# thu-nics/Rad-NeRF

Measured on AMD Instinct MI355X. Metric: million samples/s fwd+bwd, 8192 rays, model_zoo_size=2; rgb L∞ vs ref, higher is better.
Workload: dtype f16/f32

## Files before the change

rad-nerf_amd/csrc/field.hip:

```cpp
#include "rn_field.h"
#include "rn_bin.h"
#include "rn_merge.h"
#include "rn_gradform.h"
#pragma clang fp contract(off)

static int g_field_dbg = 0;
__device__ unsigned long long g_rn_cyc[8];

namespace {

template <int MODE, int CACHE>
__global__ void __launch_bounds__(256, FWD_MIN_WAVES)
k_field_fwd(FieldArgs a) {
    __shared__ __attribute__((aligned(16))) rn_half sW[FIELD_FWD_FRAGS * RN_FRAG_HALFS];
    __shared__ LvTab sT;
    const int k = blockIdx.y;
    rn_block_copy16(sW, a.frags + (size_t)k * FIELD_FRAGS * RN_FRAG_HALFS,
                    FIELD_FWD_FRAGS * RN_FRAG_BYTES);
    lv_stage(sT, a.gm);
    __syncthreads();
    int64_t base, n;
    sample_range(a, MODE, k, base, n);
    const int64_t n_tiles = (n + 31) / 32;
    const int waves = blockDim.x / RN_WAVE;
// ... 789 lines not shown
    auto eighth_g = [&](int e) -> float* {
        return e < 4 ? reinterpret_cast<float*>(sImg) + e * EB
                     : reinterpret_cast<float*>(sW) + (e - 4) * EB;
    };
    static_assert(4 * W2_RING_WORDS * 4 <= BWD_WAVES * SC_STREAMS * 3 * SC_RING * 4, "rings");
    static_assert(4 * EB * 4 + 4 * W2_RING_WORDS * 4 <= BWD_WAVES * 2 * RN_IMG_HALFS * 2,
                  "eighths 0-3 + rings in the image region");
    static_assert(4 * EB * 4 <= FIELD_FRAGS * RN_FRAG_HALFS * 2, "eighths 4-7 in the weights");
    uint32_t* ring2 = wid < 4 ? sRing + wid * W2_RING_WORDS
                              : reinterpret_cast<uint32_t*>(sImg) + 4 * EB +
                                    (wid - 4) * W2_RING_WORDS;
    float* const wG = eighth_g(rn_lane() >> 3);
    float* const wU = wG + MB_WIN * SG_STRIDE;
    bool sw_ok = false;

    f32x16 accA = rn_zero16(), accB = rn_zero16();
    DwScale cur = {0.f, 0.f};
    int cur_k = -1;
    uint64_t cyc[8] = {0, 0, 0, 0, 0, 0, 0, 0};
    float* park = m.park + (size_t)blockIdx.x * K * BWD_WAVES * 2048 + wid * 2048;
    float* rows = m.scratch + (size_t)blockIdx.x * m.rows_cap * MB_ROW;
    const __amdgpu_buffer_rsrc_t rows_rs = rn_rsrc(rows, (uint32_t)m.rows_cap * MB_ROW * 4u);
    int n_local = 0;
    int ticket = 0, n_chunks = 0;
    if (threadIdx.x == 0) {
        n_chunks = m.queue[1];
        ticket = DET ? (int)blockIdx.x : atomicAdd(m.queue, 1);
    }
    if (threadIdx.x < K) sCh[2 + 3 * MB_KMAX + threadIdx.x] = a.seg_base[threadIdx.x];

    for (;;) {
        __syncthreads();
        if (threadIdx.x == 0) {
            const int ch = ticket;
            ticket = DET ? (ch < n_chunks ? ch + (int)gridDim.x : ch) : atomicAdd(m.queue, 1);
            int4 d[CH_DESC / 4];
            if (ch < n_chunks) {
#pragma unroll
                for (int q = 0; q < CH_DESC / 4; ++q)
                    d[q] = reinterpret_cast<const int4*>(m.desc + (size_t)ch * CH_DESC)[q];
            }
            const int32_t* di = reinterpret_cast<const int32_t*>(d);
            sCh[0] = ch < n_chunks ? di[CH_R0] : B; sCh[1] = ch < n_chunks ? di[CH_R1] : B;
            int roff = 0;
            for (int k = 0; k < K; ++k) {
                const int nk = ch < n_chunks ? di[ch_count(k)] : 0;
                sCh[2 + k] = di[ch_first(k)]; sCh[2 + MB_KMAX + k] = nk;
                sCh[2 + 2 * MB_KMAX + k] = roff;
                roff += nk;
            }
        }
        __syncthreads();
        const int r0 = sCh[0], r1 = sCh[1];
        if (r0 >= B) break;
        const bool rev = n_local & 1;
        ++n_local;
        constexpr int RAYS_LDS = BWD_WAVES * SC_STREAMS * 3 * SC_RING / 6;
        const int nr_lds = r1 - r0 <= RAYS_LDS ? r1 - r0 : 0;
        float* sRays = reinterpret_cast<float*>(sRing);
        for (int i = threadIdx.x; i < 6 * nr_lds; i += blockDim.x) {
            const int q = i / 6, cc = i - 6 * q;
            sRays[i] = cc < 3 ? a.rays_o[3 * (r0 + q) + cc] : a.rays_d[3 * (r0 + q) + cc - 3];
        }
        __syncthreads();

        const bool prof = ABL && (rn_dbg(dbg) & 4096);
        uint64_t tp0 = prof ? __builtin_amdgcn_s_memtime() : 0;
        for (int kk = 0; kk < K; ++kk) {
            const int k = rev ? K - 1 - kk : kk;
            const int a_k = sCh[2 + k], n_k = sCh[2 + MB_KMAX + k], roff = sCh[2 + 2 * MB_KMAX + k];
            if (n_k == 0) continue;
            uint64_t ts0 = prof ? __builtin_amdgcn_s_memtime() : 0;
            if (k != cur_k || !sw_ok) {
                constexpr int WV = (FIELD_FRAGS * RN_FRAG_BYTES / 16 + BWD_WAVES * RN_WAVE - 1) /
                                   (BWD_WAVES * RN_WAVE);
// ... 384 lines not shown
                      gb_pool_pages >= 1),
          "binned mode needs scale, stats, the encoding cache and the page pool");
    for (int l = 0; binned && l < RN_L; ++l)
        CHECK(level_hsize[l] <= (1u << GB_IDX_BITS) &&
              level_hsize[l] <= ((uint32_t)GB_MAX_BINS << GB_SLICE_BITS),
              "binned mode: a level has more than 2^20 entries");
    CHECK(fx_mode != GM_FX_REDO || (fx_redo && fx_scale && feat_cache),
          "fixed-point redo needs the redo flag, the step's scales and the encoding cache");
    CHECK(!(igrad_lo && fx_mode), "integer and fixed-point modes are exclusive");
    CHECK(n_rays >= 1 && n_models >= 1 && n_models <= MB_KMAX && blocks >= 1 &&
          max_samples >= 1 && max_chunk >= 1, "bad sizes");
    CHECK(scratch_rows >= (int64_t)max_chunk + (int64_t)n_models * max_samples,
          "scratch_rows must be >= max_chunk + n_models * max_samples");
    CHECK(ts && ray_of && rays_o && rays_d && seg_base && seg_count && mstart && perm &&
          chunk_desc && queue && grid_f16 && level_offset && level_hsize && level_res &&
          level_scale && xyz_min && extent && frags && dL_dsigma && dL_drgb && grid_grad && dw &&
          scratch && park, "null pointer");
    CHECK(fx_mode != GM_FX ||
          2ull * ((uint64_t)level_offset[RN_L - 1] + level_hsize[RN_L - 1]) <= (1ull << 28),
          "fixed-point mode: the grid has more than 2^28 gradient elements");
#undef CHECK
    FieldArgs a{};
    field_args_grid(a, grid_f16, level_offset, level_hsize, level_res, level_scale, xyz_min, extent,
                    frags);
    field_args_compact(a, ts, ray_of, rays_o, rays_d, seg_base, seg_count);
    a.dsigma = dL_dsigma; a.drgb = dL_drgb; a.grid_grad = grid_grad; a.dw = dw;
    a.feat = (rn_half*)feat_cache;
    MergeArgs m{};
    m.mstart = mstart; m.perm = perm; m.desc = chunk_desc; m.queue = queue; m.scratch = scratch;
    m.park = park; m.rows_cap = (int)scratch_rows; m.n_rays = (int)n_rays; m.n_models = n_models;
    hipStream_t st = (hipStream_t)stream;
    const size_t slots = (size_t)blocks * n_models * FIELD_PARAMS * sizeof(float);
    if (det) RN_CHECK_HIP_AS(who, hipMemsetAsync(dw, 0, slots, st), "dw_part reset");
    else RN_CHECK_HIP_AS(who, hipMemsetAsync(queue, 0, sizeof(int32_t), st), "ticket reset");
    IntGrad G{};
    if (igrad_lo) {
        G.bytes = 2 * a.grid_bytes;
        G.lo_ptr = igrad_lo; G.carry_ptr = igrad_carry; G.scale_ptr = igrad_scale;
    }
    if (binned) {
        RN_CHECK_HIP_AS(who, hipMemsetAsync(gb_ctl, 0, GB_CTL_RESET_BYTES, st), "page pool reset");
        G.ctl = (GbCtl*)gb_ctl; G.page_meta = gb_page_meta; G.pages = gb_pages;
        G.pool_pages = (uint32_t)gb_pool_pages;
    }
    FxGrad F{};
    F.acc = fx_acc; F.scale = fx_scale; F.redo = fx_redo;
    if (FxStats* S = reinterpret_cast<FxStats*>(fx_stats)) {
        F.vmax = S->vmax; F.qsum = S->qsum; F.wq = S->wq;
    }
    const int gm = fx_mode ? fx_mode : (igrad_lo ? GM_INT : GM_F32);
    const bool abl = RN_ABL && a.dbg && !det && gm != GM_INT && gm != GM_FX_REDO;
    if (abl) launch_bwd_merged<RN_ABL != 0, 0>(gm, blocks, st, a, m, G, F);
    else if (!det) launch_bwd_merged<false, 0>(gm, blocks, st, a, m, G, F);
    else launch_bwd_merged<false, 1>(gm, blocks, st, a, m, G, F);
    RN_CHECK_LAUNCH_AS(who);
    return 0;
}

extern "C" {
int rn_field_bwd_merged(const float* ts, const int32_t* ray_of, const float* rays_o,
                        const float* rays_d, const int32_t* seg_base, const int32_t* seg_count,
                        const int32_t* mstart, const int32_t* perm, const int32_t* chunk_desc,
                        int32_t* queue, int64_t n_rays, int32_t n_models, int32_t max_samples,
                        const void* grid_f16, const uint32_t* level_offset,
                        const uint32_t* level_hsize, const uint32_t* level_res,
                        const float* level_scale, const float* xyz_min, const float* extent,
                        const void* frags, const float* dL_dsigma, const float* dL_drgb,
// ... 43 lines not shown
```

rad-nerf_amd/csrc/field_grad.hip:

```cpp
#include "rn_field.h"
#include "rn_bin.h"
#include "rn_gradform.h"
#pragma clang fp contract(off)

namespace {

__global__ void __launch_bounds__(256)
k_seed_max(const int32_t* __restrict__ seg_base, const int32_t* __restrict__ seg_count,
           const float* __restrict__ sigma, const float* __restrict__ dsigma,
           const float* __restrict__ drgb, uint32_t* __restrict__ mbits) {
    const int k = blockIdx.y;
    const int64_t base = seg_base[k], n = seg_count[k];
    float mx = 0.f;
    for (int64_t i = (int64_t)blockIdx.x * blockDim.x + threadIdx.x; i < n;
         i += (int64_t)gridDim.x * blockDim.x) {
        const int64_t s = base + i;
        mx = fmaxf(mx, fabsf(dsigma[s] * sigma[s]));
        mx = fmaxf(mx, fmaxf(fabsf(drgb[3 * s]), fmaxf(fabsf(drgb[3 * s + 1]), fabsf(drgb[3 * s + 2]))));
    }
    mx = rn_wave_max(mx);
    if (rn_lane() == 0 && mx > 0.f && isfinite(mx)) atomicMax(mbits, __float_as_uint(mx));
}

__global__ void k_seed_scale(const uint32_t* __restrict__ mbits, float* __restrict__ scale) {
    const float m = __uint_as_float(*mbits);
    float sc = 1.0f;
    if (m > 0.f) {
        int e;
        frexpf(m, &e);
        sc = scalbnf(1.0f, max(-100, min(100, 26 - e)));
    }
    *scale = sc;
}

__global__ void __launch_bounds__(256)
k_igrad_to_f32(int64_t n, int32_t* __restrict__ lo, int32_t* __restrict__ carry,
               const float* __restrict__ scale, float* __restrict__ grad) {
    const int64_t i = (int64_t)blockIdx.x * blockDim.x + threadIdx.x;
    if (i >= n) return;
    const double v = ((double)carry[i] * 4294967296.0 + (double)lo[i]) / (double)*scale;
    grad[i] += (float)v;
    lo[i] = 0;
    carry[i] = 0;
}

__global__ void __launch_bounds__(256)
k_fx_esum(GridMeta gm, const float* __restrict__ scale, const int32_t* __restrict__ acc,
          const float* __restrict__ grad, FxStats* __restrict__ st) {
    const int l = blockIdx.y;
    const float sc = scale[l];
    typedef int vi4 __attribute__((ext_vector_type(4)));
    const int64_t e0 = 2 * (int64_t)gm.offset[l], n4 = (2 * (int64_t)gm.hsize[l]) >> 2;
    int64_t s = 0;
    uint64_t ws = 0;
    uint32_t mx = 0u;
    auto uabs = [](int x) { return x < 0 ? 0u - (uint32_t)x : (uint32_t)x; };
    if (sc != 0.f) {
        const vi4* a4 = reinterpret_cast<const vi4*>(acc + e0);
        for (int64_t i = (int64_t)blockIdx.x * blockDim.x + threadIdx.x; i < n4;
             i += (int64_t)gridDim.x * blockDim.x) {
            const vi4 v = __builtin_nontemporal_load(a4 + i);
            s += (int64_t)v.x + v.y + v.z + v.w;
            const uint32_t el = (uint32_t)(e0 + 4 * i);
            ws += (uint64_t)((int64_t)v.x * (int64_t)fx_weight(el)) +
                  (uint64_t)((int64_t)v.y * (int64_t)fx_weight(el + 1)) +
                  (uint64_t)((int64_t)v.z * (int64_t)fx_weight(el + 2)) +
                  (uint64_t)((int64_t)v.w * (int64_t)fx_weight(el + 3));
            mx = max(max(mx, max(uabs(v.x), uabs(v.y))), max(uabs(v.z), uabs(v.w)));
        }
    } else {
        const vi4* g4 = reinterpret_cast<const vi4*>(grad + e0);
        for (int64_t i = (int64_t)blockIdx.x * blockDim.x + threadIdx.x; i < n4;
             i += (int64_t)gridDim.x * blockDim.x) {
            const vi4 v = __builtin_nontemporal_load(g4 + i);
            mx = max(max(mx, max((uint32_t)v.x & 0x7fffffffu, (uint32_t)v.y & 0x7fffffffu)),
                     max((uint32_t)v.z & 0x7fffffffu, (uint32_t)v.w & 0x7fffffffu));
        }
    }
#pragma unroll
    for (int off = 32; off > 0; off >>= 1) {
        s += __shfl_xor(s, off);
        ws += __shfl_xor(ws, off);
        mx = max(mx, (uint32_t)__shfl_xor((int)mx, off));
    }
    __shared__ int64_t sW[4];
    __shared__ uint64_t sWw[4];
    __shared__ uint32_t sM[4];
    const int w = threadIdx.x / RN_WAVE;
    if (rn_lane() == 0) { sW[w] = s; sWw[w] = ws; sM[w] = mx; }
    __syncthreads();
    if (threadIdx.x == 0) {
        const int64_t t = (sW[0] + sW[1]) + (sW[2] + sW[3]);
        const uint64_t tw = (sWw[0] + sWw[1]) + (sWw[2] + sWw[3]);
        if (tw != 0) atomicAdd(reinterpret_cast<unsigned long long*>(st->we + l), tw);
        uint32_t m = max(max(sM[0], sM[1]), max(sM[2], sM[3]));
        if (sc != 0.f) m = __float_as_uint((float)m / sc);
        if (t != 0) atomicAdd(reinterpret_cast<unsigned long long*>(st->esum + l), (unsigned long long)t);
        if (m != 0u && m < 0x7f800000u) atomicMax(st->emax + l, m);
    }
}

#ifndef FX_TARGET_BITS
#define FX_TARGET_BITS 27
#endif
#ifndef FX_ENTRY_BITS
#define FX_ENTRY_BITS 29
#endif
#define FX_DENSE_FIRST_BITS 14
#ifndef FX_GROWTH_BITS
#define FX_GROWTH_BITS 30
#endif
#define FX_GROWTH_UNITS ((float)(1u << FX_GROWTH_BITS))
__global__ void __launch_bounds__(64)
k_fx_check(uint32_t hashed_mask, const float* __restrict__ scale_cur,
           float* __restrict__ scale_next, FxStats* __restrict__ stats,
           int32_t* __restrict__ redo, const GbCtl* __restrict__ ctl, uint32_t pool_pages) {
    const int l = threadIdx.x;
    uint32_t* vmax = stats->vmax;
    const bool binned = ctl != nullptr;
    bool bad = binned && l == 0 && (ctl->pool_next > pool_pages || ctl->fault != 0u);
    const float growth = binned ? GB_GROWTH_UNITS : FX_GROWTH_UNITS;
    if (l < RN_L) {
        if (!binned && scale_cur[l] != 0.f &&
            (stats->esum[l] != stats->qsum[l] || stats->we[l] != stats->wq[l]))
            bad = true;
        stats->esum[l] = 0;
        stats->qsum[l] = 0;
        stats->we[l] = 0;
        stats->wq[l] = 0;
        const uint32_t vb = vmax[l];
        const float sc = scale_cur[l];
        const uint32_t em = stats->emax[l];
        float nx = sc;
        if (vb >= 0x7f800000u) {
            nx = 0.f;
            bad = bad || sc != 0.f;
        } else if (vb != 0u) {
            const float v = __uint_as_float(vb);
            bad = bad || (sc != 0.f && v * sc >= growth);
            int e;
            frexpf(v, &e);
            int bits = (binned ? GB_TARGET_BITS : FX_TARGET_BITS) - e;
            if (binned) {
            } else if (em != 0u) {
                int ee;
                frexpf(__uint_as_float(em), &ee);
                bits = min(bits, FX_ENTRY_BITS - ee);
            } else if (!((hashed_mask >> l) & 1u)) {
                bits = FX_DENSE_FIRST_BITS - e;
            }
            nx = scalbnf(1.0f, max(-126, min(126, bits)));
        }
        scale_next[l] = nx;
        vmax[l] = 0u;
        stats->emax[l] = 0u;
    }
    const uint64_t b = __builtin_amdgcn_ballot_w64(bad);
    if (l == 0) *redo = b ? 1 : 0;
}

__global__ void __launch_bounds__(256)
k_fx_fold(int64_t e0, int64_t e1, GridMeta gm, const float* __restrict__ scale,
          int32_t* __restrict__ acc, float* __restrict__ grad, const int32_t* __restrict__ redo) {
    __shared__ uint32_t sOff[RN_L];
    __shared__ float sInv[RN_L];
    if (threadIdx.x < RN_L) {
        sOff[threadIdx.x] = gm.offset[threadIdx.x];
        const float sc = scale[threadIdx.x];
        sInv[threadIdx.x] = sc != 0.f ? 1.0f / sc : 0.f;
    }
    __syncthreads();
    const bool discard = *redo != 0;
    const int64_t n4 = (e1 - e0) >> 2;
    typedef int vi4 __attribute__((ext_vector_type(4)));
    vi4* a4 = reinterpret_cast<vi4*>(acc + e0);
    float4* g4 = reinterpret_cast<float4*>(grad + e0);
    for (int64_t i = (int64_t)blockIdx.x * blockDim.x + threadIdx.x; i < n4;
         i += (int64_t)gridDim.x * blockDim.x) {
        const vi4 v = __builtin_nontemporal_load(a4 + i);
        if ((v.x | v.y | v.z | v.w) == 0) continue;
        __builtin_nontemporal_store(vi4{0, 0, 0, 0}, a4 + i);
        if (discard) continue;
        const uint32_t ent = (uint32_t)((e0 + 4 * i) >> 1);
        int l = 0;
#pragma unroll
        for (int k = 1; k < RN_L; ++k) l = ent >= sOff[k] ? k : l;
        const float inv = sInv[l];
        float4 g = g4[i];
        g.x += (float)v.x * inv; g.y += (float)v.y * inv;
        g.z += (float)v.z * inv; g.w += (float)v.w * inv;
        g4[i] = g;
    }
}
// ... 5 lines not shown
int rn_seed_scale(const int32_t* seg_base, const int32_t* seg_count, int32_t n_models,
                  const float* sigma, const float* dL_dsigma, const float* dL_drgb,
                  uint32_t* work, float* scale, void* stream) {
    RN_CHECK_ARG(n_models >= 1, "bad sizes");
    RN_CHECK_ARG(seg_base && seg_count && sigma && dL_dsigma && dL_drgb && work && scale,
                 "null pointer");
    hipStream_t st = (hipStream_t)stream;
    RN_CHECK_HIP(hipMemsetAsync(work, 0, sizeof(uint32_t), st), "memset");
    k_seed_max<<<dim3(256, n_models), 256, 0, st>>>(seg_base, seg_count, sigma, dL_dsigma,
                                                     dL_drgb, work);
    RN_CHECK_LAUNCH();
    k_seed_scale<<<1, 1, 0, st>>>(work, scale);
    RN_CHECK_LAUNCH();
    return 0;
}

int rn_grid_fx_fold(const uint32_t* level_offset, const uint32_t* level_hsize,
                    const uint32_t* level_res, int32_t* fx_acc, const float* fx_scale_cur,
                    float* fx_scale_next, uint32_t* fx_vmax, int32_t* fx_redo, float* grid_grad,
                    void* stream) {
    RN_CHECK_ARG(level_offset && level_hsize && level_res && fx_acc && fx_scale_cur &&
                 fx_scale_next && fx_vmax && fx_redo && grid_grad, "null pointer");
    RN_CHECK_ARG(fx_scale_cur != fx_scale_next, "scale_cur and scale_next must differ");
    GridMeta gm{};
    uint32_t hashed = 0;
    for (int l = 0; l < RN_L; ++l) {
        gm.offset[l] = level_offset[l]; gm.hsize[l] = level_hsize[l]; gm.res[l] = level_res[l];
        const uint64_t r = level_res[l];
        if (r * r * r > (uint64_t)level_hsize[l]) hashed |= 1u << l;
        RN_CHECK_ARG(level_offset[l] % 8 == 0, "level offsets must be multiples of 8 entries");
    }
    hipStream_t st = (hipStream_t)stream;
    FxStats* stats = reinterpret_cast<FxStats*>(fx_vmax);
    k_fx_esum<<<dim3(128, RN_L), 256, 0, st>>>(gm, fx_scale_cur, fx_acc, grid_grad, stats);
    k_fx_check<<<1, 64, 0, st>>>(hashed, fx_scale_cur, fx_scale_next, stats, fx_redo, nullptr, 0u);
    RN_CHECK_LAUNCH();
    {
        const int64_t e0 = 2 * (int64_t)level_offset[0];
        const int64_t e1 = 2 * ((int64_t)level_offset[RN_L - 1] + level_hsize[RN_L - 1]);
        RN_CHECK_ARG(e1 % 4 == 0, "table size must be a multiple of 2 entries");
        const int64_t n4 = (e1 - e0) / 4;
        const int nb = (int)std::min<int64_t>(2048, (n4 + 255) / 256);
        k_fx_fold<<<nb > 0 ? nb : 1, 256, 0, st>>>(e0, e1, gm, fx_scale_cur, fx_acc, grid_grad,
                                                    fx_redo);
        RN_CHECK_LAUNCH();
    }
    return 0;
}

}

int rn_fx_check_binned(const float* fx_scale_cur, float* fx_scale_next, uint32_t* fx_stats,
                       int32_t* fx_redo, const void* ctl, uint32_t pool_pages, void* stream) {
    k_fx_check<<<1, 64, 0, (hipStream_t)stream>>>(0u, fx_scale_cur, fx_scale_next,
                                                  reinterpret_cast<FxStats*>(fx_stats), fx_redo,
                                                  (const GbCtl*)ctl, pool_pages);
    RN_CHECK_LAUNCH();
    return 0;
}

extern "C" {

int rn_igrad_to_f32(int64_t n, int32_t* igrad_lo, int32_t* igrad_carry, const float* scale,
                    float* grid_grad, void* stream) {
    RN_CHECK_ARG(n >= 0, "bad size");
    if (n == 0) return 0;
    RN_CHECK_ARG(igrad_lo && igrad_carry && scale && grid_grad, "null pointer");
    k_igrad_to_f32<<<nblk(n, 256), 256, 0, (hipStream_t)stream>>>(n, igrad_lo, igrad_carry, scale,
// ... 7 lines not shown
```

rad-nerf_amd/csrc/field_plan.hip:

```cpp
#include "rn_field.h"
#include "rn_merge.h"
#pragma clang fp contract(off)

namespace {

#define PLAN_WAVES 4
#define PLAN_LDS 2048

#define PLAN_UNR 8

struct PlanPrep {
    float4* prep;
    const float* rays_o; const float* rays_d;
    float mn[3], ext[3];
    float inv[3];
};
struct RayPos { float o[3], d[3]; };
__device__ __forceinline__ RayPos plan_ray(const PlanPrep& P, int r) {
    RayPos q;
#pragma unroll
    for (int c = 0; c < 3; ++c) { q.o[c] = P.rays_o[3 * r + c]; q.d[c] = P.rays_d[3 * r + c]; }
    return q;
}
__device__ __forceinline__ void plan_prep_write(const PlanPrep& P, const RayPos& q, int pos,
// ... 19 lines not shown
    ms = 0;
#pragma unroll
    for (int k = 0; k < MB_KMAX; ++k) {
        cnt[k] = k < K ? c[k] : 0;
        off[k] = k < K ? o[k] : 0;
        ms += k < K ? o[k] - sb[k] : 0;
    }
}
__device__ __forceinline__ void plan_stage(int K, int tot_r, const int* bnd, const int* off,
                                           const float* __restrict__ ts, float* st, uint16_t* si) {
    const int lane = rn_lane();
    for (int i0 = 0; i0 < tot_r; i0 += RN_WAVE * PLAN_UNR) {
        float v[PLAN_UNR];
#pragma unroll
        for (int u = 0; u < PLAN_UNR; ++u) {
            const int i = i0 + u * RN_WAVE + lane;
            int base = off[0];
#pragma unroll
            for (int kq = 1; kq < MB_KMAX; ++kq)
                base = (kq < K && i >= bnd[kq]) ? off[kq] - bnd[kq] : base;
            v[u] = i < tot_r ? ts[base + i] : 0.f;
        }
#pragma unroll
        for (int u = 0; u < PLAN_UNR; ++u) {
            const int i = i0 + u * RN_WAVE + lane;
            if (i < tot_r) {
                st[i] = v[u];
                if (si) si[i] = (uint16_t)i;
            }
        }
    }
}

__global__ void __launch_bounds__(PLAN_WAVES * 64)
k_bwd_plan(int B, int K, const int32_t* __restrict__ counts, const int32_t* __restrict__ offsets,
           const int32_t* __restrict__ seg_base, const int32_t* __restrict__ seg_count,
           const float* __restrict__ ts, int32_t* __restrict__ mstart, int32_t* __restrict__ perm,
           PlanPrep P) {
    __shared__ float sT[PLAN_WAVES][PLAN_LDS];
    const int wid = __builtin_amdgcn_readfirstlane(threadIdx.x / RN_WAVE);
    const int r = blockIdx.x * PLAN_WAVES + wid;
    if (r >= B) return;
    const int lane = rn_lane();
    int ms = 0, tot_r = 0;
    int cnt[MB_KMAX], off[MB_KMAX], loc[MB_KMAX];
    plan_ray_runs(K, B, r, counts, offsets, seg_base, cnt, off, ms);
#pragma unroll
    for (int k = 0; k < MB_KMAX; ++k) { loc[k] = tot_r; tot_r += cnt[k]; }
    if (lane == 0) {
        mstart[r] = ms;
        if (r == 0) {
            int tot = 0;
            for (int k = 0; k < K; ++k) tot += seg_count[k];
            mstart[B] = tot;
        }
    }
    const bool staged = tot_r <= PLAN_LDS;
    float* st = sT[wid];
    const RayPos rq = P.prep ? plan_ray(P, r) : RayPos{};
    if (staged) {
        plan_stage(K, tot_r, loc, off, ts, st, nullptr);
        __builtin_amdgcn_wave_barrier();
        __builtin_amdgcn_fence(__ATOMIC_ACQ_REL, "wavefront");
    }
    if (K == 2 && staged) {
        const float* A = st + loc[0];
        const float* Bv = st + loc[1];
        const int nA = cnt[0], nB = cnt[1], n = nA + nB;
        const int L = (n + RN_WAVE - 1) / RN_WAVE;
        const int d = min(lane * L, n);
        int lo = max(0, d - nB), hi = min(d, nA);
        while (lo < hi) {
// ... 46 lines not shown
    const int d = min(lane * L, n);
    int lo = max(0, d - nB), hi = min(d, nA);
    while (lo < hi) {
        const int mid = (lo + hi) >> 1;
        if (tA[mid] <= tB[d - 1 - mid]) lo = mid + 1; else hi = mid;
    }
    int a = lo, b = d - lo;
    const int e = min(d + L, n);
    for (int q = d; q < e; ++q) {
        const float ta = tA[a], tb = tB[b];
        const int ja = iA[a], jb = iB[b];
        const bool takeA = a < nA && (b >= nB || ta <= tb);
        const int idx = takeA ? ja : jb;
        if (gout) {
            int base = ko[0];
#pragma unroll
            for (int j = 1; j < MB_KMAX; ++j)
                if (j < K && idx >= kb[j]) base = ko[j] - kb[j];
            gout[q] = base + idx;
            if (P.prep) plan_prep_write(P, rq, gpos + q, takeA ? ta : tb, base + idx);
        } else {
            to[q] = takeA ? ta : tb;
            io[q] = (uint16_t)idx;
        }
        a += takeA ? 1 : 0;
        b += takeA ? 0 : 1;
    }
}

__global__ void __launch_bounds__(PLANM_WAVES * 64)
k_bwd_plan_multi(int B, int K, const int32_t* __restrict__ counts,
                 const int32_t* __restrict__ offsets, const int32_t* __restrict__ seg_base,
                 const int32_t* __restrict__ seg_count, const float* __restrict__ ts,
                 int32_t* __restrict__ mstart, int32_t* __restrict__ perm, PlanPrep P) {
    __shared__ float sT[PLANM_WAVES][2][PLANM_LDS + 2];
    __shared__ uint16_t sI[PLANM_WAVES][2][PLANM_LDS + 2];
    static_assert(PLANM_LDS <= 65536, "u16 sample ids");
    const int wid = __builtin_amdgcn_readfirstlane(threadIdx.x / RN_WAVE);
    const int r = blockIdx.x * PLANM_WAVES + wid;
    if (r >= B) return;
    const int lane = rn_lane();
    int ms = 0, tot_r = 0;
    int bnd[MB_KMAX + 1], off[MB_KMAX], cnt[MB_KMAX];
    plan_ray_runs(K, B, r, counts, offsets, seg_base, cnt, off, ms);
#pragma unroll
    for (int k = 0; k < MB_KMAX; ++k) { bnd[k] = tot_r; tot_r += cnt[k]; }
    bnd[MB_KMAX] = tot_r;
    const RayPos rq = P.prep ? plan_ray(P, r) : RayPos{};
    if (lane == 0) {
        mstart[r] = ms;
        if (r == 0) {
            int tot = 0;
            for (int k = 0; k < K; ++k) tot += seg_count[k];
            mstart[B] = tot;
        }
    }
    if (tot_r > PLANM_LDS) {
        for (int k = 0; k < K; ++k) {
            const int ck = bnd[k + 1] - bnd[k];
            for (int i = lane; i < ck; i += RN_WAVE) {
                const float t = ts[off[k] + i];
                int pos = i;
                for (int k2 = 0; k2 < K; ++k2) {
                    if (k2 == k) continue;
                    int lo = 0, hi = bnd[k2 + 1] - bnd[k2];
                    while (lo < hi) {
                        const int mid = (lo + hi) >> 1;
                        const float t2 = ts[off[k2] + mid];
                        if (t2 < t || (k2 < k && t2 == t)) lo = mid + 1; else hi = mid;
                    }
// ... 14 lines not shown
    while (true) {
        __builtin_amdgcn_wave_barrier();
        __builtin_amdgcn_fence(__ATOMIC_ACQ_REL, "wavefront");
        const bool last = nr <= 2;
        const float* ts_ = sT[wid][cur];
        const uint16_t* is_ = sI[wid][cur];
        for (int p = 0; 2 * p < nr; ++p) {
            const int a0 = bnd[2 * p], a1 = bnd[min(2 * p + 1, nr)], b1 = bnd[min(2 * p + 2, nr)];
            merge_pair_wave(ts_ + a0, is_ + a0, a1 - a0, ts_ + a1, is_ + a1, b1 - a1,
                            sT[wid][cur ^ 1] + a0, sI[wid][cur ^ 1] + a0,
                            nullptr, kb, off, K, P, rq, ms + a0);
        }
        if (last) {
            __builtin_amdgcn_wave_barrier();
            __builtin_amdgcn_fence(__ATOMIC_ACQ_REL, "wavefront");
            const float* to = sT[wid][cur ^ 1];
            const uint16_t* io = sI[wid][cur ^ 1];
            for (int q = lane; q < tot_r; q += RN_WAVE) {
                const int idx = io[q];
                int base = off[0];
#pragma unroll
                for (int jk = 1; jk < MB_KMAX; ++jk)
                    if (jk < K && idx >= kb[jk]) base = off[jk] - kb[jk];
                perm[ms + q] = base + idx;
                if (P.prep) plan_prep_write(P, rq, ms + q, to[q], base + idx);
            }
            return;
        }
        const int nn = (nr + 1) / 2;
        for (int p = 0; p < nn; ++p) bnd[p] = bnd[2 * p];
        bnd[nn] = bnd[nr];
        nr = nn;
        cur ^= 1;
    }
}

struct ChunkPlan {
    int head_n, head, max_chunk, min_chunk, c1, n;
    __host__ __device__ int hbound(int c) const {
        return head_n > 0 ? (int)(((int64_t)head * c * (c + 1)) / (2 * (int64_t)head_n)) : 0;
    }
    __host__ __device__ int bound(int c) const {
        const int H = hbound(head_n);
        if (c < head_n) return hbound(c);
        if (c <= c1) return H + (c - head_n) * max_chunk;
        return H + (c1 - head_n) * max_chunk + (c - c1) * min_chunk;
    }
};

__host__ __device__ __forceinline__ ChunkPlan chunk_plan(int total, int head_n, int head,
                                                         int max_chunk, int min_chunk, int blocks) {
    ChunkPlan p;
    p.head = head; p.max_chunk = max_chunk; p.min_chunk = min_chunk;
#ifndef RN_TAIL_SHIFT
#define RN_TAIL_SHIFT 4
#endif
    static_assert(RN_TAIL_SHIFT >= 3, "the documented cap_chunks bound assumes a tail <= 1/8");
    const int main_end = total - (RN_TAIL_SHIFT < 31 ? total >> RN_TAIL_SHIFT : 0);
    p.head_n = head > 0 && (int64_t)head * (head_n + 1) / 2 <= main_end ? head_n : 0;
    const int H = p.hbound(p.head_n);
    if (blocks > 0 && main_end > H) {
        const int64_t main = main_end - H, per = (int64_t)blocks * max_chunk;
        const int64_t m = (main + per - 1) / per;
        const int64_t sz = (main + (int64_t)blocks * m - 1) / ((int64_t)blocks * m);
        p.max_chunk = (int)(sz < min_chunk ? min_chunk : (sz > max_chunk ? max_chunk : sz));
    }
    p.c1 = p.head_n + (main_end > H ? (main_end - H) / p.max_chunk : 0);
    const int rest = total - p.bound(p.c1);
    p.n = p.c1 + (rest > 0 ? (rest + min_chunk - 1) / min_chunk : 0);
    return p;
}

__global__ void __launch_bounds__(256)
k_bwd_chunks(int B, int K, const int32_t* __restrict__ mstart,
             const int32_t* __restrict__ offsets, const int32_t* __restrict__ seg_base,
             const int32_t* __restrict__ seg_count, int head_n, int head, int max_chunk,
             int min_chunk, int blocks, int cap_chunks, int32_t* __restrict__ chunk_first,
             int32_t* __restrict__ desc, int32_t* __restrict__ queue) {
    const int c = blockIdx.x * blockDim.x + threadIdx.x;
    const int total = mstart[B];
    const ChunkPlan p = chunk_plan(total, head_n, head, max_chunk, min_chunk, blocks);
    const int n = min(p.n, cap_chunks);
    if (c == 0) { queue[0] = 0; queue[1] = n; queue[2] = 0; }
    if (c > n) return;
    auto first_ray = [&](int cc) {
        if (cc == p.n) return B;
        const int bound = p.bound(cc);
        int lo = 0, hi = B;
        while (lo < hi) {
            const int mid = (lo + hi) >> 1;
            if (mstart[mid] < bound) lo = mid + 1; else hi = mid;
        }
        return lo;
    };
    if (c == n) { chunk_first[c] = first_ray(c); return; }
    const int first[2] = {first_ray(c), first_ray(c + 1)};
    chunk_first[c] = first[0];
    int32_t* d = desc + (size_t)c * CH_DESC;
    const int r0 = first[0], r1 = first[1];
    d[CH_R0] = r0; d[CH_R1] = r1; d[2] = 0; d[3] = 0;
    for (int k = 0; k < MB_KMAX; ++k) {
        int a0 = 0, cnt = 0;
        if (k < K && r0 < B) {
            a0 = offsets[k * B + r0];
            const int a1 = r1 < B ? offsets[k * B + r1] : seg_base[k] + seg_count[k];
            cnt = a1 - a0;
        }
        d[ch_first(k)] = a0; d[ch_count(k)] = cnt;
    }
}

}

extern "C" {

int rn_bwd_plan(const int32_t* counts, const int32_t* offsets, const int32_t* seg_base,
                const int32_t* seg_count, const float* ts, int64_t n_rays, int32_t n_models,
                int32_t head_chunks, int32_t head_size, int32_t max_chunk, int32_t min_chunk,
                int32_t balance_blocks, int32_t cap_chunks, int32_t* mstart, int32_t* perm,
                int32_t* chunk_first, int32_t* chunk_desc, int32_t* queue, const float* rays_o,
                const float* rays_d, const float* xyz_min, const float* extent, float* prep,
                void* stream) {
    RN_CHECK_ARG(n_rays >= 1 && n_models >= 1 && n_models <= MB_KMAX, "bad sizes");
    RN_CHECK_ARG(max_chunk >= min_chunk && min_chunk >= 1 && cap_chunks >= 1 && head_chunks >= 0 &&
                 head_size >= 0 && head_size <= max_chunk && balance_blocks >= 0,
                 "bad chunk sizes");
    RN_CHECK_ARG(counts && offsets && seg_base && seg_count && ts && mstart && perm &&
                 chunk_first && chunk_desc && queue, "null pointer");
    RN_CHECK_ARG(!prep || (rays_o && rays_d && xyz_min && extent), "null pointer (prep)");
    PlanPrep P{};
    P.prep = (float4*)prep; P.rays_o = rays_o; P.rays_d = rays_d;
    if (prep) {
        bool pow2 = true;
        for (int c = 0; c < 3; ++c) {
            P.mn[c] = xyz_min[c]; P.ext[c] = extent[c];
            int e;
            pow2 = pow2 && extent[c] > 0.f && std::frexp(extent[c], &e) == 0.5f &&
                   e > -120 && e < 120;
        }
        for (int c = 0; c < 3; ++c) P.inv[c] = pow2 ? 1.0f / extent[c] : 0.f;
    }
    if (n_models > 2)
        k_bwd_plan_multi<<<nblk(n_rays, PLANM_WAVES), PLANM_WAVES * 64, 0, (hipStream_t)stream>>>(
            (int)n_rays, n_models, counts, offsets, seg_base, seg_count, ts, mstart, perm, P);
    else
        k_bwd_plan<<<nblk(n_rays, PLAN_WAVES), PLAN_WAVES * 64, 0, (hipStream_t)stream>>>(
            (int)n_rays, n_models, counts, offsets, seg_base, seg_count, ts, mstart, perm, P);
    RN_CHECK_LAUNCH();
    k_bwd_chunks<<<nblk(cap_chunks + 1, 256), 256, 0, (hipStream_t)stream>>>(
        (int)n_rays, n_models, mstart, offsets, seg_base, seg_count, head_chunks, head_size,
        max_chunk, min_chunk, balance_blocks, cap_chunks, chunk_first, chunk_desc, queue);
    RN_CHECK_LAUNCH();
    return 0;
}

}
```

Baseline: 1218.

## Fuse planning and fixed-point check kernels, drop ticket reset memset

Three launches are removed. The chunk-planning kernel is folded into the plan kernel as extra blocks; these recompute the prefix from per-model offsets instead of reading mstart. The fx check runs in the last-arriving block of a widened, unrolled esum kernel through an arrival counter. The ticket-queue memset is replaced by the last ticket-taking block resetting the counter itself. The aim is to cut launch and serialization overhead on the small fwd+bwd step, at the cost of subtle cross-block synchronization and ordering risks.

Result: no change. 1224 (median of 6 runs) (+0.5%).

```diff
diff --git a/rad-nerf_amd/csrc/field.hip b/rad-nerf_amd/csrc/field.hip
--- a/rad-nerf_amd/csrc/field.hip
+++ b/rad-nerf_amd/csrc/field.hip
@@ -845,15 +845,19 @@
     for (;;) {
         __syncthreads();
         if (threadIdx.x == 0) {
-            const int ch = ticket;
-            ticket = DET ? (ch < n_chunks ? ch + (int)gridDim.x : ch) : atomicAdd(m.queue, 1);
+            int ch;
             int4 d[CH_DESC / 4];
-            if (ch < n_chunks) {
+            const int32_t* di = reinterpret_cast<const int32_t*>(d);
+            for (;;) {
+                ch = ticket;
+                ticket = DET ? (ch < n_chunks ? ch + (int)gridDim.x : ch) : atomicAdd(m.queue, 1);
+                if (!DET && ticket == n_chunks + 2 * (int)gridDim.x - 1) atomicExch(m.queue, 0);
+                if (ch >= n_chunks) break;
 #pragma unroll
                 for (int q = 0; q < CH_DESC / 4; ++q)
                     d[q] = reinterpret_cast<const int4*>(m.desc + (size_t)ch * CH_DESC)[q];
-            }
-            const int32_t* di = reinterpret_cast<const int32_t*>(d);
+                if (di[CH_R0] < B) break;
+            }
             sCh[0] = ch < n_chunks ? di[CH_R0] : B; sCh[1] = ch < n_chunks ? di[CH_R1] : B;
             int roff = 0;
             for (int k = 0; k < K; ++k) {
@@ -1304,7 +1308,6 @@
     hipStream_t st = (hipStream_t)stream;
     const size_t slots = (size_t)blocks * n_models * FIELD_PARAMS * sizeof(float);
     if (det) RN_CHECK_HIP_AS(who, hipMemsetAsync(dw, 0, slots, st), "dw_part reset");
-    else RN_CHECK_HIP_AS(who, hipMemsetAsync(queue, 0, sizeof(int32_t), st), "ticket reset");
     IntGrad G{};
     if (igrad_lo) {
         G.bytes = 2 * a.grid_bytes;
diff --git a/rad-nerf_amd/csrc/field_grad.hip b/rad-nerf_amd/csrc/field_grad.hip
--- a/rad-nerf_amd/csrc/field_grad.hip
+++ b/rad-nerf_amd/csrc/field_grad.hip
@@ -1,3 +1,4 @@
+#include <atomic>
 #include "rn_field.h"
 #include "rn_bin.h"
 #include "rn_gradform.h"
@@ -44,9 +45,29 @@
     carry[i] = 0;
 }
 
-__global__ void __launch_bounds__(256)
-k_fx_esum(GridMeta gm, const float* __restrict__ scale, const int32_t* __restrict__ acc,
-          const float* __restrict__ grad, FxStats* __restrict__ st) {
+#ifndef FX_ESUM_BLOCKS
+#define FX_ESUM_BLOCKS 24
+#endif
+#ifndef FX_ESUM_THREADS
+#define FX_ESUM_THREADS 1024
+#endif
+#ifndef FX_ESUM_UNR
+#define FX_ESUM_UNR 4
+#endif
+#define FX_ESUM_WAVES (FX_ESUM_THREADS / RN_WAVE)
+#define FX_ARRIVE_SLOTS 64
+__device__ uint32_t g_fx_arrive[FX_ARRIVE_SLOTS];
+
+__device__ __forceinline__ void fx_check_wave(uint32_t hashed_mask,
+                                              const float* __restrict__ scale_cur,
+                                              float* __restrict__ scale_next, FxStats* stats,
+                                              int32_t* __restrict__ redo, const GbCtl* ctl,
+                                              uint32_t pool_pages);
+
+__global__ void __launch_bounds__(FX_ESUM_THREADS)
+k_fx_esum(GridMeta gm, uint32_t hashed_mask, const float* __restrict__ scale,
+          float* __restrict__ scale_next, const int32_t* __restrict__ acc,
+          const float* __restrict__ grad, FxStats* st, int32_t* __restrict__ redo, int slot) {
     const int l = blockIdx.y;
     const float sc = scale[l];
     typedef int vi4 __attribute__((ext_vector_type(4)));
@@ -55,26 +76,36 @@
     uint64_t ws = 0;
     uint32_t mx = 0u;
     auto uabs = [](int x) { return x < 0 ? 0u - (uint32_t)x : (uint32_t)x; };
-    if (sc != 0.f) {
-        const vi4* a4 = reinterpret_cast<const vi4*>(acc + e0);
-        for (int64_t i = (int64_t)blockIdx.x * blockDim.x + threadIdx.x; i < n4;
-             i += (int64_t)gridDim.x * blockDim.x) {
-            const vi4 v = __builtin_nontemporal_load(a4 + i);
-            s += (int64_t)v.x + v.y + v.z + v.w;
-            const uint32_t el = (uint32_t)(e0 + 4 * i);
-            ws += (uint64_t)((int64_t)v.x * (int64_t)fx_weight(el)) +
-                  (uint64_t)((int64_t)v.y * (int64_t)fx_weight(el + 1)) +
-                  (uint64_t)((int64_t)v.z * (int64_t)fx_weight(el + 2)) +
-                  (uint64_t)((int64_t)v.w * (int64_t)fx_weight(el + 3));
-            mx = max(max(mx, max(uabs(v.x), uabs(v.y))), max(uabs(v.z), uabs(v.w)));
+    const int64_t stride = (int64_t)gridDim.x * blockDim.x;
+    const vi4* t4 = reinterpret_cast<const vi4*>(sc != 0.f ? (const void*)(acc + e0)
+                                                           : (const void*)(grad + e0));
+    for (int64_t i0 = (int64_t)blockIdx.x * blockDim.x + threadIdx.x; i0 < n4;
+         i0 += FX_ESUM_UNR * stride) {
+        vi4 v[FX_ESUM_UNR];
+#pragma unroll
+        for (int u = 0; u < FX_ESUM_UNR; ++u) {
+            const int64_t i = i0 + u * stride;
+            v[u] = i < n4 ? t4[i] : vi4{0, 0, 0, 0};
         }
-    } else {
-        const vi4* g4 = reinterpret_cast<const vi4*>(grad + e0);
-        for (int64_t i = (int64_t)blockIdx.x * blockDim.x + threadIdx.x; i < n4;
-             i += (int64_t)gridDim.x * blockDim.x) {
-            const vi4 v = __builtin_nontemporal_load(g4 + i);
-            mx = max(max(mx, max((uint32_t)v.x & 0x7fffffffu, (uint32_t)v.y & 0x7fffffffu)),
-                     max((uint32_t)v.z & 0x7fffffffu, (uint32_t)v.w & 0x7fffffffu));
+        if (sc != 0.f) {
+#pragma unroll
+            for (int u = 0; u < FX_ESUM_UNR; ++u) {
+                const vi4 q = v[u];
+                s += (int64_t)q.x + q.y + q.z + q.w;
+                const uint32_t el = (uint32_t)(e0 + 4 * (i0 + u * stride));
+                ws += (uint64_t)((int64_t)q.x * (int64_t)fx_weight(el)) +
+                      (uint64_t)((int64_t)q.y * (int64_t)fx_weight(el + 1)) +
+                      (uint64_t)((int64_t)q.z * (int64_t)fx_weight(el + 2)) +
+                      (uint64_t)((int64_t)q.w * (int64_t)fx_weight(el + 3));
+                mx = max(max(mx, max(uabs(q.x), uabs(q.y))), max(uabs(q.z), uabs(q.w)));
+            }
+        } else {
+#pragma unroll
+            for (int u = 0; u < FX_ESUM_UNR; ++u) {
+                const vi4 q = v[u];
+                mx = max(max(mx, max((uint32_t)q.x & 0x7fffffffu, (uint32_t)q.y & 0x7fffffffu)),
+                         max((uint32_t)q.z & 0x7fffffffu, (uint32_t)q.w & 0x7fffffffu));
+            }
         }
     }
 #pragma unroll
@@ -83,21 +114,37 @@
         ws += __shfl_xor(ws, off);
         mx = max(mx, (uint32_t)__shfl_xor((int)mx, off));
     }
-    __shared__ int64_t sW[4];
-    __shared__ uint64_t sWw[4];
-    __shared__ uint32_t sM[4];
-    const int w = threadIdx.x / RN_WAVE;
+    __shared__ int64_t sW[FX_ESUM_WAVES];
+    __shared__ uint64_t sWw[FX_ESUM_WAVES];
+    __shared__ uint32_t sM[FX_ESUM_WAVES];
+    const int w = __builtin_amdgcn_readfirstlane(threadIdx.x / RN_WAVE);
     if (rn_lane() == 0) { sW[w] = s; sWw[w] = ws; sM[w] = mx; }
     __syncthreads();
+    if (w != 0) return;
+    int last = 0;
     if (threadIdx.x == 0) {
-        const int64_t t = (sW[0] + sW[1]) + (sW[2] + sW[3]);
-        const uint64_t tw = (sWw[0] + sWw[1]) + (sWw[2] + sWw[3]);
+        int64_t t = 0;
+        uint64_t tw = 0;
+        uint32_t m = 0u;
+#pragma unroll
+        for (int q = 0; q < FX_ESUM_WAVES; ++q) { t += sW[q]; tw += sWw[q]; m = max(m, sM[q]); }
         if (tw != 0) atomicAdd(reinterpret_cast<unsigned long long*>(st->we + l), tw);
-        uint32_t m = max(max(sM[0], sM[1]), max(sM[2], sM[3]));
         if (sc != 0.f) m = __float_as_uint((float)m / sc);
         if (t != 0) atomicAdd(reinterpret_cast<unsigned long long*>(st->esum + l), (unsigned long long)t);
         if (m != 0u && m < 0x7f800000u) atomicMax(st->emax + l, m);
-    }
+        asm volatile("s_waitcnt vmcnt(0)" ::: "memory");
+        __builtin_amdgcn_fence(__ATOMIC_RELEASE, "agent");
+        asm volatile("s_waitcnt vmcnt(0)" ::: "memory");
+        const uint32_t nblocks = gridDim.x * gridDim.y;
+        last = __hip_atomic_fetch_add(g_fx_arrive + slot, 1u, __ATOMIC_RELAXED,
+                                      __HIP_MEMORY_SCOPE_AGENT) == nblocks - 1u;
+        if (last) __hip_atomic_store(g_fx_arrive + slot, 0u, __ATOMIC_RELAXED,
+                                     __HIP_MEMORY_SCOPE_AGENT);
+    }
+    last = __builtin_amdgcn_readfirstlane(last);
+    if (!last) return;
+    __builtin_amdgcn_fence(__ATOMIC_ACQUIRE, "agent");
+    fx_check_wave(hashed_mask, scale, scale_next, st, redo, nullptr, 0u);
 }
 
 #ifndef FX_TARGET_BITS
@@ -111,11 +158,12 @@
 #define FX_GROWTH_BITS 30
 #endif
 #define FX_GROWTH_UNITS ((float)(1u << FX_GROWTH_BITS))
-__global__ void __launch_bounds__(64)
-k_fx_check(uint32_t hashed_mask, const float* __restrict__ scale_cur,
-           float* __restrict__ scale_next, FxStats* __restrict__ stats,
-           int32_t* __restrict__ redo, const GbCtl* __restrict__ ctl, uint32_t pool_pages) {
-    const int l = threadIdx.x;
+__device__ __forceinline__ void fx_check_wave(uint32_t hashed_mask,
+                                              const float* __restrict__ scale_cur,
+                                              float* __restrict__ scale_next, FxStats* stats,
+                                              int32_t* __restrict__ redo, const GbCtl* ctl,
+                                              uint32_t pool_pages) {
+    const int l = rn_lane();
     uint32_t* vmax = stats->vmax;
     const bool binned = ctl != nullptr;
     bool bad = binned && l == 0 && (ctl->pool_next > pool_pages || ctl->fault != 0u);
@@ -159,6 +207,13 @@
     if (l == 0) *redo = b ? 1 : 0;
 }
 
+__global__ void __launch_bounds__(64)
+k_fx_check(uint32_t hashed_mask, const float* __restrict__ scale_cur,
+           float* __restrict__ scale_next, FxStats* __restrict__ stats,
+           int32_t* __restrict__ redo, const GbCtl* __restrict__ ctl, uint32_t pool_pages) {
+    fx_check_wave(hashed_mask, scale_cur, scale_next, stats, redo, ctl, pool_pages);
+}
+
 __global__ void __launch_bounds__(256)
 k_fx_fold(int64_t e0, int64_t e1, GridMeta gm, const float* __restrict__ scale,
           int32_t* __restrict__ acc, float* __restrict__ grad, const int32_t* __restrict__ redo) {
@@ -230,8 +285,10 @@
     }
     hipStream_t st = (hipStream_t)stream;
     FxStats* stats = reinterpret_cast<FxStats*>(fx_vmax);
-    k_fx_esum<<<dim3(128, RN_L), 256, 0, st>>>(gm, fx_scale_cur, fx_acc, grid_grad, stats);
-    k_fx_check<<<1, 64, 0, st>>>(hashed, fx_scale_cur, fx_scale_next, stats, fx_redo, nullptr, 0u);
+    static std::atomic<unsigned> next_slot{0};
+    const int slot = (int)(next_slot.fetch_add(1u, std::memory_order_relaxed) % FX_ARRIVE_SLOTS);
+    k_fx_esum<<<dim3(FX_ESUM_BLOCKS, RN_L), FX_ESUM_THREADS, 0, st>>>(gm, hashed, fx_scale_cur, fx_scale_next,
+                                                          fx_acc, grid_grad, stats, fx_redo, slot);
     RN_CHECK_LAUNCH();
     {
         const int64_t e0 = 2 * (int64_t)level_offset[0];
diff --git a/rad-nerf_amd/csrc/field_plan.hip b/rad-nerf_amd/csrc/field_plan.hip
--- a/rad-nerf_amd/csrc/field_plan.hip
+++ b/rad-nerf_amd/csrc/field_plan.hip
@@ -75,12 +75,98 @@
     }
 }
 
+struct ChunkPlan {
+    int head_n, head, max_chunk, min_chunk, c1, n;
+    __host__ __device__ int hbound(int c) const {
+        return head_n > 0 ? (int)(((int64_t)head * c * (c + 1)) / (2 * (int64_t)head_n)) : 0;
+    }
+    __host__ __device__ int bound(int c) const {
+        const int H = hbound(head_n);
+        if (c < head_n) return hbound(c);
+        if (c <= c1) return H + (c - head_n) * max_chunk;
+        return H + (c1 - head_n) * max_chunk + (c - c1) * min_chunk;
+    }
+};
+
+__host__ __device__ __forceinline__ ChunkPlan chunk_plan(int total, int head_n, int head,
+                                                         int max_chunk, int min_chunk, int blocks) {
+    ChunkPlan p;
+    p.head = head; p.max_chunk = max_chunk; p.min_chunk = min_chunk;
+#ifndef RN_TAIL_SHIFT
+#define RN_TAIL_SHIFT 4
+#endif
+    static_assert(RN_TAIL_SHIFT >= 3, "the documented cap_chunks bound assumes a tail <= 1/8");
+    const int main_end = total - (RN_TAIL_SHIFT < 31 ? total >> RN_TAIL_SHIFT : 0);
+    p.head_n = head > 0 && (int64_t)head * (head_n + 1) / 2 <= main_end ? head_n : 0;
+    const int H = p.hbound(p.head_n);
+    if (blocks > 0 && main_end > H) {
+        const int64_t main = main_end - H, per = (int64_t)blocks * max_chunk;
+        const int64_t m = (main + per - 1) / per;
+        const int64_t sz = (main + (int64_t)blocks * m - 1) / ((int64_t)blocks * m);
+        p.max_chunk = (int)(sz < min_chunk ? min_chunk : (sz > max_chunk ? max_chunk : sz));
+    }
+    p.c1 = p.head_n + (main_end > H ? (main_end - H) / p.max_chunk : 0);
+    const int rest = total - p.bound(p.c1);
+    p.n = p.c1 + (rest > 0 ? (rest + min_chunk - 1) / min_chunk : 0);
+    return p;
+}
+
+struct ChunkArgs {
+    int plan_blocks;
+    int head_n, head, max_chunk, min_chunk, blocks, cap_chunks;
+    int32_t* chunk_first; int32_t* desc; int32_t* queue;
+};
+__device__ __forceinline__ void plan_chunks(int B, int K, const int32_t* __restrict__ offsets,
+                                            const int32_t* __restrict__ seg_base,
+                                            const int32_t* __restrict__ seg_count,
+                                            const ChunkArgs& C, int c) {
+    int total = 0, sb = 0;
+    for (int k = 0; k < K; ++k) { total += seg_count[k]; sb += seg_base[k]; }
+    const ChunkPlan p = chunk_plan(total, C.head_n, C.head, C.max_chunk, C.min_chunk, C.blocks);
+    const int n = min(p.n, C.cap_chunks);
+    if (c == 0) { C.queue[0] = 0; C.queue[1] = n; C.queue[2] = 0; }
+    if (c > n) return;
+    auto first_ray = [&](int cc) {
+        if (cc == p.n) return B;
+        const int bound = p.bound(cc);
+        int lo = 0, hi = B;
+        while (lo < hi) {
+            const int mid = (lo + hi) >> 1;
+            int ms = -sb;
+#pragma unroll
+            for (int k = 0; k < MB_KMAX; ++k) ms += k < K ? offsets[k * B + mid] : 0;
+            if (ms < bound) lo = mid + 1; else hi = mid;
+        }
+        return lo;
+    };
+    if (c == n) { C.chunk_first[c] = first_ray(c); return; }
+    const int first[2] = {first_ray(c), first_ray(c + 1)};
+    C.chunk_first[c] = first[0];
+    int32_t* d = C.desc + (size_t)c * CH_DESC;
+    const int r0 = first[0], r1 = first[1];
+    d[CH_R0] = r0; d[CH_R1] = r1; d[2] = 0; d[3] = 0;
+    for (int k = 0; k < MB_KMAX; ++k) {
+        int a0 = 0, cnt = 0;
+        if (k < K && r0 < B) {
+            a0 = offsets[k * B + r0];
+            const int a1 = r1 < B ? offsets[k * B + r1] : seg_base[k] + seg_count[k];
+            cnt = a1 - a0;
+        }
+        d[ch_first(k)] = a0; d[ch_count(k)] = cnt;
+    }
+}
+
 __global__ void __launch_bounds__(PLAN_WAVES * 64)
 k_bwd_plan(int B, int K, const int32_t* __restrict__ counts, const int32_t* __restrict__ offsets,
            const int32_t* __restrict__ seg_base, const int32_t* __restrict__ seg_count,
            const float* __restrict__ ts, int32_t* __restrict__ mstart, int32_t* __restrict__ perm,
-           PlanPrep P) {
+           PlanPrep P, ChunkArgs C) {
     __shared__ float sT[PLAN_WAVES][PLAN_LDS];
+    if ((int)blockIdx.x >= C.plan_blocks) {
+        plan_chunks(B, K, offsets, seg_base, seg_count, C,
+                    ((int)blockIdx.x - C.plan_blocks) * PLAN_WAVES * 64 + (int)threadIdx.x);
+        return;
+    }
     const int wid = __builtin_amdgcn_readfirstlane(threadIdx.x / RN_WAVE);
     const int r = blockIdx.x * PLAN_WAVES + wid;
     if (r >= B) return;
@@ -193,10 +279,16 @@
 k_bwd_plan_multi(int B, int K, const int32_t* __restrict__ counts,
                  const int32_t* __restrict__ offsets, const int32_t* __restrict__ seg_base,
                  const int32_t* __restrict__ seg_count, const float* __restrict__ ts,
-                 int32_t* __restrict__ mstart, int32_t* __restrict__ perm, PlanPrep P) {
+                 int32_t* __restrict__ mstart, int32_t* __restrict__ perm, PlanPrep P,
+                 ChunkArgs C) {
     __shared__ float sT[PLANM_WAVES][2][PLANM_LDS + 2];
     __shared__ uint16_t sI[PLANM_WAVES][2][PLANM_LDS + 2];
     static_assert(PLANM_LDS <= 65536, "u16 sample ids");
+    if ((int)blockIdx.x >= C.plan_blocks) {
+        plan_chunks(B, K, offsets, seg_base, seg_count, C,
+                    ((int)blockIdx.x - C.plan_blocks) * PLANM_WAVES * 64 + (int)threadIdx.x);
+        return;
+    }
     const int wid = __builtin_amdgcn_readfirstlane(threadIdx.x / RN_WAVE);
     const int r = blockIdx.x * PLANM_WAVES + wid;
     if (r >= B) return;
@@ -277,81 +369,6 @@
         bnd[nn] = bnd[nr];
         nr = nn;
         cur ^= 1;
-    }
-}
-
-struct ChunkPlan {
-    int head_n, head, max_chunk, min_chunk, c1, n;
-    __host__ __device__ int hbound(int c) const {
-        return head_n > 0 ? (int)(((int64_t)head * c * (c + 1)) / (2 * (int64_t)head_n)) : 0;
-    }
-    __host__ __device__ int bound(int c) const {
-        const int H = hbound(head_n);
-        if (c < head_n) return hbound(c);
-        if (c <= c1) return H + (c - head_n) * max_chunk;
-        return H + (c1 - head_n) * max_chunk + (c - c1) * min_chunk;
-    }
-};
-
-__host__ __device__ __forceinline__ ChunkPlan chunk_plan(int total, int head_n, int head,
-                                                         int max_chunk, int min_chunk, int blocks) {
-    ChunkPlan p;
-    p.head = head; p.max_chunk = max_chunk; p.min_chunk = min_chunk;
-#ifndef RN_TAIL_SHIFT
-#define RN_TAIL_SHIFT 4
-#endif
-    static_assert(RN_TAIL_SHIFT >= 3, "the documented cap_chunks bound assumes a tail <= 1/8");
-    const int main_end = total - (RN_TAIL_SHIFT < 31 ? total >> RN_TAIL_SHIFT : 0);
-    p.head_n = head > 0 && (int64_t)head * (head_n + 1) / 2 <= main_end ? head_n : 0;
-    const int H = p.hbound(p.head_n);
-    if (blocks > 0 && main_end > H) {
-        const int64_t main = main_end - H, per = (int64_t)blocks * max_chunk;
-        const int64_t m = (main + per - 1) / per;
-        const int64_t sz = (main + (int64_t)blocks * m - 1) / ((int64_t)blocks * m);
-        p.max_chunk = (int)(sz < min_chunk ? min_chunk : (sz > max_chunk ? max_chunk : sz));
-    }
-    p.c1 = p.head_n + (main_end > H ? (main_end - H) / p.max_chunk : 0);
-    const int rest = total - p.bound(p.c1);
-    p.n = p.c1 + (rest > 0 ? (rest + min_chunk - 1) / min_chunk : 0);
-    return p;
-}
-
-__global__ void __launch_bounds__(256)
-k_bwd_chunks(int B, int K, const int32_t* __restrict__ mstart,
-             const int32_t* __restrict__ offsets, const int32_t* __restrict__ seg_base,
-             const int32_t* __restrict__ seg_count, int head_n, int head, int max_chunk,
-             int min_chunk, int blocks, int cap_chunks, int32_t* __restrict__ chunk_first,
-             int32_t* __restrict__ desc, int32_t* __restrict__ queue) {
-    const int c = blockIdx.x * blockDim.x + threadIdx.x;
-    const int total = mstart[B];
-    const ChunkPlan p = chunk_plan(total, head_n, head, max_chunk, min_chunk, blocks);
-    const int n = min(p.n, cap_chunks);
-    if (c == 0) { queue[0] = 0; queue[1] = n; queue[2] = 0; }
-    if (c > n) return;
-    auto first_ray = [&](int cc) {
-        if (cc == p.n) return B;
-        const int bound = p.bound(cc);
-        int lo = 0, hi = B;
-        while (lo < hi) {
-            const int mid = (lo + hi) >> 1;
-            if (mstart[mid] < bound) lo = mid + 1; else hi = mid;
-        }
-        return lo;
-    };
-    if (c == n) { chunk_first[c] = first_ray(c); return; }
-    const int first[2] = {first_ray(c), first_ray(c + 1)};
-    chunk_first[c] = first[0];
-    int32_t* d = desc + (size_t)c * CH_DESC;
-    const int r0 = first[0], r1 = first[1];
-    d[CH_R0] = r0; d[CH_R1] = r1; d[2] = 0; d[3] = 0;
-    for (int k = 0; k < MB_KMAX; ++k) {
-        int a0 = 0, cnt = 0;
-        if (k < K && r0 < B) {
-            a0 = offsets[k * B + r0];
-            const int a1 = r1 < B ? offsets[k * B + r1] : seg_base[k] + seg_count[k];
-            cnt = a1 - a0;
-        }
-        d[ch_first(k)] = a0; d[ch_count(k)] = cnt;
     }
 }
 
@@ -385,16 +402,21 @@
         }
         for (int c = 0; c < 3; ++c) P.inv[c] = pow2 ? 1.0f / extent[c] : 0.f;
     }
-    if (n_models > 2)
-        k_bwd_plan_multi<<<nblk(n_rays, PLANM_WAVES), PLANM_WAVES * 64, 0, (hipStream_t)stream>>>(
-            (int)n_rays, n_models, counts, offsets, seg_base, seg_count, ts, mstart, perm, P);
-    else
-        k_bwd_plan<<<nblk(n_rays, PLAN_WAVES), PLAN_WAVES * 64, 0, (hipStream_t)stream>>>(
-            (int)n_rays, n_models, counts, offsets, seg_base, seg_count, ts, mstart, perm, P);
-    RN_CHECK_LAUNCH();
-    k_bwd_chunks<<<nblk(cap_chunks + 1, 256), 256, 0, (hipStream_t)stream>>>(
-        (int)n_rays, n_models, mstart, offsets, seg_base, seg_count, head_chunks, head_size,
-        max_chunk, min_chunk, balance_blocks, cap_chunks, chunk_first, chunk_desc, queue);
+    ChunkArgs C{};
+    C.head_n = head_chunks; C.head = head_size; C.max_chunk = max_chunk; C.min_chunk = min_chunk;
+    C.blocks = balance_blocks; C.cap_chunks = cap_chunks;
+    C.chunk_first = chunk_first; C.desc = chunk_desc; C.queue = queue;
+    if (n_models > 2) {
+        C.plan_blocks = nblk(n_rays, PLANM_WAVES);
+        k_bwd_plan_multi<<<C.plan_blocks + nblk(cap_chunks + 1, PLANM_WAVES * 64), PLANM_WAVES * 64,
+                           0, (hipStream_t)stream>>>(
+            (int)n_rays, n_models, counts, offsets, seg_base, seg_count, ts, mstart, perm, P, C);
+    } else {
+        C.plan_blocks = nblk(n_rays, PLAN_WAVES);
+        k_bwd_plan<<<C.plan_blocks + nblk(cap_chunks + 1, PLAN_WAVES * 64), PLAN_WAVES * 64, 0,
+                     (hipStream_t)stream>>>(
+            (int)n_rays, n_models, counts, offsets, seg_base, seg_count, ts, mstart, perm, P, C);
+    }
     RN_CHECK_LAUNCH();
     return 0;
 }
```
